# coecms/xmhw

Hardware: AMD Instinct MI355X
Metric: grid-cells/sec for threshold() on 40yr daily SST (higher is better)
Workload: dtype f32 in / f64 out; 1 GPU; 0.25deg global (configs[2]): 1036800 cells per step, 1982-2021 (T=14610), windowHalfWidth=5, pctile=90, smoothPercentileWidth=31, nan_frac=0.0, skipna=False; cells_rank0=1036800, T=14610, D=366, kernel=clim_sorted_f32 (sorted row-lists in LDS, 2 lanes per cell, layout 40), slabs=1, gather=none

## Files before the change

include/xmhw_amd.h:

```cpp
#ifndef XMHW_AMD_H
#define XMHW_AMD_H

#include <stddef.h>
#include <stdint.h>

#ifdef __cplusplus
extern "C" {
#endif

#define XMHW_OK 0
#define XMHW_ERR_INVALID 1
#define XMHW_ERR_HIP 2
#define XMHW_ERR_UNSUPPORTED 3
#define XMHW_ERR_NOMEM 4
#define XMHW_ERR_COMM 5

#define XMHW_KERNEL_AUTO 0
#define XMHW_KERNEL_RING 1
#define XMHW_KERNEL_GENERIC 2

int xmhw_version(void);
const char *xmhw_arch(void);
const char *xmhw_last_error(void);
int xmhw_device_count(int *count);
// ... 39 lines not shown
int xmhw_event_elapsed_ms(void *start, void *stop, float *ms);

typedef struct xmhw_plan xmhw_plan;

int xmhw_plan_create(const int32_t *doy_host, int64_t T, int32_t window_half_width,
                     xmhw_plan **plan);
int xmhw_plan_destroy(xmhw_plan *plan);
int xmhw_plan_info(const xmhw_plan *plan, int32_t *D, int32_t *ntracks,
                   int32_t *kernel, int32_t *nsteps, int32_t *step_min);
int xmhw_plan_doys(const xmhw_plan *plan, int32_t *doys_out );
int xmhw_plan_set_kernel(xmhw_plan *plan, int32_t kernel);
int xmhw_plan_set_narrowing(xmhw_plan *plan, int32_t enable);
int xmhw_plan_set_timing(xmhw_plan *plan, int32_t enable);
int xmhw_plan_kernel_ms(xmhw_plan *plan, int32_t calls_back, float *ms);
int xmhw_plan_narrowed(xmhw_plan *plan, int32_t *narrowed_out);
int xmhw_plan_set_chunks(xmhw_plan *plan, int32_t nchunks);
int xmhw_plan_chunks_in_use(const xmhw_plan *plan, int64_t C, int32_t *nchunks);
int xmhw_plan_table(const xmhw_plan *plan, int32_t years_per_lane, uint32_t *table_out,
                    int32_t *ntracks_padded);
int xmhw_plan_sorted_info(const xmhw_plan *plan, int64_t C, int32_t *keys_per_list, int32_t *lds_bytes_per_wave,
                          int32_t *pieces);
int xmhw_plan_sorted_table(const xmhw_plan *plan, int32_t pieces, int32_t *nchunks, int32_t *nrows, int32_t *ntp,
                           int32_t *chunks_out, uint32_t *table_out, uint32_t *flags_out);

int xmhw_debug_stats_available(void);
int xmhw_plan_debug_stats_n(xmhw_plan *plan, int enable, uint64_t *out, int32_t n);
int xmhw_plan_debug_stats(xmhw_plan *plan, int enable, uint64_t *out8);

enum {
    XMHW_LAYOUT_AUTO = -2,
    XMHW_LAYOUT_RING1 = -1,
    XMHW_LAYOUT_RING2_8LANE = 8,
    XMHW_LAYOUT_RING2_4LANE = 10,
    XMHW_LAYOUT_RING2_16LANE = 12,
    XMHW_LAYOUT_RING3_8LANE = 20,
    XMHW_LAYOUT_RING3_4LANE = 21,
    XMHW_LAYOUT_RING3_2LANE = 22,
    XMHW_LAYOUT_SORTED = 40
};
int xmhw_plan_set_layout(xmhw_plan *plan, int32_t layout);
int xmhw_plan_layout_in_use(const xmhw_plan *plan, int32_t *layout);
int xmhw_sorted_device_ok(int32_t *holds);
int xmhw_plan_set_ring2(xmhw_plan *plan, int32_t variant);
int xmhw_plan_ring2_in_use(const xmhw_plan *plan, int32_t *variant);
int xmhw_plan_f64_mode(const xmhw_plan *plan, int32_t *variant);
enum { XMHW_ROUTE_GENERIC = 0, XMHW_ROUTE_RING1 = 1, XMHW_ROUTE_RING2 = 2, XMHW_ROUTE_RING3 = 3, XMHW_ROUTE_RING4 = 4,
// ... 488 lines not shown
```

xmhw_amd/csrc/capi.cpp:

```cpp
#include "../../include/xmhw_amd.h"

#include <hip/hip_runtime.h>
#include <unistd.h>

#include <cerrno>
#include <cmath>

#include <algorithm>
#include <cstdio>
#include <cstdlib>
#include <atomic>
#include <cstring>
#include <map>
#include <memory>
#include <mutex>
#include <new>
#include <string>
#include <vector>

#include "kernels.h"
#include "plan.h"
#include "route.h"
#include "stage_blocks.h"

// ... 17 lines not shown
namespace {
#define HIP_TRY(expr)                                        \
    do {                                                     \
        hipError_t _e = (expr);                              \
        if (_e != hipSuccess) return hip_fail(_e, #expr);    \
    } while (0)

constexpr int kSubs = 8;

}

struct PlanDevice {
    int32_t* row_ptr = nullptr;
    int32_t* centres = nullptr;
    uint32_t* sflags = nullptr;
    xmhw::DevChunk* chunks = nullptr;
    int32_t nchunks = 0;
    unsigned long long* stats = nullptr;
    uint32_t* narrow_flag = nullptr;
    uint32_t* table_s = nullptr;
    uint32_t* sflags_s = nullptr;
    xmhw::DevSortedChunk* chunks_s = nullptr;
    int32_t nchunks_s = 0;
};

struct xmhw_plan {
    xmhw::Plan host;
    xmhw::RouteSettings settings = xmhw::route_defaults();
    std::mutex mu;
    bool uploaded = false;
    PlanDevice dev;
    std::map<std::pair<int32_t, int32_t>, uint32_t*> tables;
    int32_t chunks_cut = 0;
    int32_t yps_s = 0;
    int64_t sorted_pieces = -1;
    bool timing = false;
    hipEvent_t tev[32] = {};
    uint64_t tcalls = 0;

    ~xmhw_plan() {
        for (hipEvent_t e : tev) if (e) (void)hipEventDestroy(e);
        for (auto& kv : tables) if (kv.second) (void)hipFree(kv.second);
        for (void* p : std::initializer_list<void*>{dev.row_ptr, dev.centres, dev.sflags, dev.chunks, dev.stats,
                                                    dev.narrow_flag, dev.table_s, dev.sflags_s, dev.chunks_s})
            if (p) (void)hipFree(p);
    }
// ... 27 lines not shown
        r = xmhw::resolve_route(p->host, p->settings, elem_bytes, q, false);
    return r;
}
xmhw::Route plan_route(const xmhw_plan* p, int elem_bytes, double q = 1.0) {
    return xmhw::resolve_route(p->host, p->settings, elem_bytes, q, true);
}

template <typename E>
hipError_t put(E** dst, const std::vector<E>& v) {
    const bool fresh = *dst == nullptr;
    hipError_t e = fresh ? hipMalloc(reinterpret_cast<void**>(dst), sizeof(E) * v.size()) : hipSuccess;
    if (e != hipSuccess) { *dst = nullptr; return e; }
    e = hipMemcpy(*dst, v.data(), sizeof(E) * v.size(), hipMemcpyHostToDevice);
    if (e != hipSuccess && fresh) { (void)hipFree(*dst); *dst = nullptr; }
    return e;
}

struct Ready {
    PlanDevice dev;
    const uint32_t* table[3] = {};
    hipEvent_t t0 = nullptr, t1 = nullptr;
};

int ensure_sorted(xmhw_plan* p, const xmhw::Launch& l, int64_t pieces) {
    PlanDevice& d = p->dev;
    if (d.table_s && p->yps_s == l.tpl && p->sorted_pieces == pieces) return XMHW_OK;
    HIP_TRY(hipDeviceSynchronize());
    for (void** q : {reinterpret_cast<void**>(&d.table_s), reinterpret_cast<void**>(&d.sflags_s),
                     reinterpret_cast<void**>(&d.chunks_s)})
        if (*q) { HIP_TRY(hipFree(*q)); *q = nullptr; }
    const xmhw::Plan::SortedPlan sp = p->host.sorted_plan(l.lanes * l.tpl, 24, pieces);
    if (sp.chunks.empty()) return fail(XMHW_ERR_UNSUPPORTED, "the sorted-list kernel has no chunks for this plan");
    std::vector<xmhw::DevSortedChunk> cs(sp.chunks.size());
    for (size_t i = 0; i < cs.size(); ++i) cs[i] = {sp.chunks[i].warm_start, sp.chunks[i].begin, sp.chunks[i].end, sp.chunks[i].trow0};
    std::stable_sort(cs.begin(), cs.end(), [](const xmhw::DevSortedChunk& a, const xmhw::DevSortedChunk& b) {
        return a.end - a.warm_start > b.end - b.warm_start;
    });
    p->sorted_pieces = -1;
    HIP_TRY(put(&d.table_s, sp.table));
    HIP_TRY(put(&d.sflags_s, sp.flags));
    HIP_TRY(put(&d.chunks_s, cs));
    d.nchunks_s = static_cast<int32_t>(cs.size());
    p->yps_s = l.tpl;
    p->sorted_pieces = pieces;
    return XMHW_OK;
}

int ensure(xmhw_plan* p, const xmhw::Route& route, int64_t C, bool timed, Ready* out) {
    std::lock_guard<std::mutex> lock(p->mu);
    const xmhw::Plan& h = p->host;
    PlanDevice& d = p->dev;
    if (!p->uploaded) {
        HIP_TRY(put(&d.row_ptr, h.row_ptr));
        HIP_TRY(put(&d.centres, h.centres));
        HIP_TRY(put(&d.sflags, h.step_flags()));
        p->uploaded = true;
    }
// ... 54 lines not shown
    if (l.family == xmhw::Family::Ring2)
        return xmhw::launch_ring2_f32_narrowing(ts, C, ld, h.T, table, rd.sflags, h.step_min, rd.chunks, rd.nchunks, h.w,
                                                l.tpl, h.ntracks, l.layout, q, negate, thresh, seas, ldo, st, rd.narrow_flag);
    if (l.family == xmhw::Family::Ring3)
        return xmhw::launch_ring3_f32_narrowing(ts, C, ld, h.T, table, rd.sflags, h.step_min, rd.chunks, rd.nchunks, h.w,
                                                l.tpl, l.lanes, h.ntracks, q, negate, thresh, seas, ldo, st, rd.narrow_flag);
    return hipErrorInvalidValue;
}

template <typename T>
hipError_t launch_one(const xmhw::Plan& h, const xmhw::Launch& l, const PlanDevice& rd, const uint32_t* table, const T* ts,
                      int64_t C, int64_t ld, double q, int negate, double* thresh, double* seas, int64_t ldo,
                      hipStream_t st) {
    using xmhw::Family;
    const uint32_t* run_flag = l.gated ? rd.narrow_flag : nullptr;
    unsigned long long* stats = l.counters ? rd.stats : nullptr;
    if (l.family == Family::Generic)
        return xmhw::launch_generic<T>(ts, h.T, C, ld, rd.row_ptr, rd.centres, h.D, h.w, q, negate, thresh, seas, ldo, st,
                                       run_flag);
    if constexpr (sizeof(T) == 4) {
        switch (l.family) {
            case Family::Sorted:
                return xmhw::launch_sorted_f32(ts, C, ld, h.T, table, rd.sflags_s, rd.chunks_s, rd.nchunks_s, h.w, l.tpl,
                                               h.ntracks, q, negate, thresh, seas, ldo, st, stats);
            case Family::Ring1:
                return xmhw::launch_ring_f32(ts, C, ld, table, h.step_min, rd.chunks, rd.nchunks, h.w, l.tpl, l.lanes, q,
                                             negate, thresh, seas, ldo, st, stats);
            case Family::Ring2:
                return xmhw::launch_ring2_f32(ts, C, ld, h.T, table, rd.sflags, h.step_min, rd.chunks, rd.nchunks, h.w, l.tpl,
                                              h.ntracks, l.layout, q, negate, thresh, seas, ldo, st, stats);
            case Family::Ring3:
                return xmhw::launch_ring3_f32(ts, C, ld, h.T, table, rd.sflags, h.step_min, rd.chunks, rd.nchunks, h.w, l.tpl,
                                              l.lanes, h.ntracks, q, negate, thresh, seas, ldo, st, stats);
#ifdef XMHW_RING4
            case Family::Ring4:
                return xmhw::launch_ring4_f32(ts, C, ld, h.T, table, rd.sflags, h.step_min, rd.chunks, rd.nchunks, h.w, l.tpl,
                                              l.lanes, h.ntracks, q, negate, thresh, seas, ldo, st, stats);
#endif
            default: return hipErrorInvalidValue;
        }
    } else {
        if (l.narrows) return launch_narrowing(h, l, rd, table, ts, C, ld, q, negate, thresh, seas, ldo, st);
        if (l.family == Family::Ring2)
            return xmhw::launch_ring2_f64(ts, C, ld, h.T, table, rd.sflags, h.step_min, rd.chunks, rd.nchunks, h.w, l.tpl,
                                          h.ntracks, l.layout, q, negate, thresh, seas, ldo, st, run_flag);
        if (l.family == Family::Ring3)
            return xmhw::launch_ring3_f64(ts, C, ld, h.T, table, rd.sflags, h.step_min, rd.chunks, rd.nchunks, h.w, l.tpl,
// ... 1367 lines not shown
}

int xmhw_plan_sorted_table(const xmhw_plan* plan, int32_t pieces, int32_t* nchunks, int32_t* nrows, int32_t* ntp,
                           int32_t* chunks_out, uint32_t* table_out, uint32_t* flags_out) {
    if (!plan) return fail(XMHW_ERR_INVALID, "plan is NULL");
    const int32_t yps = xmhw::sorted_pick_yps(plan->host.w, plan->host.ntracks);
    if (yps == 0) return fail(XMHW_ERR_UNSUPPORTED, "the sorted-list kernel is not instantiated for this window / record length");
    const xmhw::Plan::SortedPlan sp = plan->host.sorted_plan(2 * yps, 24, std::max(pieces, 1));
    if (nchunks) *nchunks = static_cast<int32_t>(sp.chunks.size());
    if (nrows) *nrows = static_cast<int32_t>(sp.flags.size());
    if (ntp) *ntp = 2 * yps;
    if (chunks_out)
        for (size_t i = 0; i < sp.chunks.size(); ++i) {
            chunks_out[4 * i + 0] = sp.chunks[i].warm_start;
            chunks_out[4 * i + 1] = sp.chunks[i].begin;
            chunks_out[4 * i + 2] = sp.chunks[i].end;
            chunks_out[4 * i + 3] = sp.chunks[i].trow0;
        }
    if (table_out) std::memcpy(table_out, sp.table.data(), sizeof(uint32_t) * sp.table.size());
    if (flags_out) std::memcpy(flags_out, sp.flags.data(), sizeof(uint32_t) * sp.flags.size());
    return XMHW_OK;
}

int xmhw_clim_raw_f32(xmhw_plan* plan, const float* ts, int64_t C, int64_t ld, double q, int negate,
                      double* thresh, double* seas, int64_t ldo, void* stream) {
    return clim_raw<float>(plan, ts, C, ld, q, negate, thresh, seas, ldo, stream);
}
int xmhw_clim_raw_f64(xmhw_plan* plan, const double* ts, int64_t C, int64_t ld, double q, int negate,
                      double* thresh, double* seas, int64_t ldo, void* stream) {
    return clim_raw<double>(plan, ts, C, ld, q, negate, thresh, seas, ldo, stream);
}

int xmhw_clim_raw_i16(xmhw_plan* plan, const int16_t* codes, int64_t C, int64_t ld, int big_endian, int has_scale,
                      double scale_factor, double add_offset, int has_fill, int32_t fill_code, int decoded_itemsize, double q,
                      int negate, double* thresh, double* seas, int64_t ldo, void* stream) {
    if (!plan) return fail(XMHW_ERR_INVALID, "plan is NULL");
    if (C < 0 || ld < C || ldo < C) return fail(XMHW_ERR_INVALID, "bad C/ld/ldo");
    if (!(q >= 0.0 && q <= 1.0)) return fail(XMHW_ERR_INVALID, "quantile must be in [0, 1]");
    if (decoded_itemsize != 4 && decoded_itemsize != 8) return fail(XMHW_ERR_INVALID, "decoded_itemsize must be 4 or 8");
    if (has_scale && !(scale_factor == scale_factor && add_offset == add_offset && scale_factor != 0.0))
        return fail(XMHW_ERR_INVALID, "scale_factor must be a non-zero number, add_offset a number");
    if (C == 0) return XMHW_OK;
    if (!codes || !thresh || !seas) return fail(XMHW_ERR_INVALID, "NULL device buffer");
    const xmhw::Route route = call_route(plan, 4, q);
    if (!route.n || route.launch[0].family != xmhw::Family::Sorted)
        return fail(XMHW_ERR_UNSUPPORTED, "packed input runs on the sorted-list kernel only (w = 5, 9..48 tracks, quantile >= 0.85 or <= 0.15): "
// ... 932 lines not shown
```

xmhw_amd/csrc/kernels.h:

```cpp
#pragma once
#include <hip/hip_runtime.h>
#include <stdint.h>

namespace xmhw {

struct DevChunk { int32_t warm_start, begin, end; };
struct PackedI16 {
    int32_t mode = 0;
    int32_t fill = 0x7FFFFFFF;
    int32_t swap = 0;
    int32_t key_neg = 0;
    int32_t val_neg = 0;
    float sf = 1.0f, of = 0.0f;
    double s = 1.0, o = 0.0;
};
struct DevSortedChunk { int32_t warm_start, begin, end, trow0; };

template <typename T>
hipError_t launch_generic(const T* ts, int64_t Tn, int64_t C, int64_t ld, const int32_t* row_ptr,
                          const int32_t* centres, int32_t D, int32_t w, double q, int negate,
                          double* thresh, double* seas, int64_t ldo, hipStream_t stream,
                          const uint32_t* run_flag = nullptr);

bool ring_supported(int32_t w, int32_t yps, int32_t subs, int elem_bytes);
int32_t ring_pick(int32_t w, int32_t ntracks, int elem_bytes, int32_t* subs_out);
hipError_t launch_ring_f32(const float* ts, int64_t C, int64_t ld, const uint32_t* table,
                           int32_t step_min, const DevChunk* chunks, int32_t nchunks,
                           int32_t w, int32_t yps, int32_t subs, double q, int negate, double* thresh,
                           double* seas, int64_t ldo, hipStream_t stream,
                           unsigned long long* stats = nullptr);

int32_t ring2_pick_yps(int32_t w, int32_t ntracks, int32_t variant);
bool ring2_narrowing_supported(int32_t w, int32_t yps, int32_t variant);
hipError_t launch_narrow_probe(const double* ts, int64_t Tn, int64_t C, int64_t ld, uint32_t* narrow_flag, hipStream_t stream);
hipError_t launch_ring2_f32_narrowing(const double* ts, int64_t C, int64_t ld, int64_t Tn, const uint32_t* table,
                                      const uint32_t* sflags, int32_t step_min, const DevChunk* chunks,
                                      int32_t nchunks, int32_t w, int32_t yps, int32_t ntracks, int32_t variant,
                                      double q, int negate, double* thresh, double* seas, int64_t ldo,
                                      hipStream_t stream, uint32_t* narrow_flag);
// ... 5 lines not shown
                            double* thresh, double* seas, int64_t ldo, hipStream_t stream, const uint32_t* run_flag);
bool ring_stats_built();
hipError_t launch_ring2_f32(const float* ts, int64_t C, int64_t ld, int64_t Tn, const uint32_t* table,
                            const uint32_t* sflags, int32_t step_min, const DevChunk* chunks, int32_t nchunks,
                            int32_t w, int32_t yps, int32_t ntracks, int32_t variant, double q, int negate,
                            double* thresh, double* seas, int64_t ldo, hipStream_t stream,
                            unsigned long long* stats = nullptr);

int32_t ring3_pick_yps(int32_t w, int32_t ntracks, int32_t subs);
bool ring3_supported(int32_t w, int32_t yps, int32_t subs);
hipError_t launch_ring3_f32(const float* ts, int64_t C, int64_t ld, int64_t Tn, const uint32_t* table,
                            const uint32_t* sflags, int32_t step_min, const DevChunk* chunks, int32_t nchunks,
                            int32_t w, int32_t yps, int32_t subs, int32_t ntracks, double q, int negate,
                            double* thresh, double* seas, int64_t ldo, hipStream_t stream,
                            unsigned long long* stats = nullptr);

int32_t sorted_pick_yps(int32_t w, int32_t ntracks);
int32_t sorted_pick_k(int32_t w, int32_t ntracks);
int32_t sorted_lds_bytes(int32_t w, int32_t ntracks);
hipError_t sorted_lds_probe(uint32_t* d_bad, hipStream_t stream);
hipError_t launch_sorted_f32(const float* ts, int64_t C, int64_t ld, int64_t Tn, const uint32_t* table,
                             const uint32_t* sflags, const DevSortedChunk* chunks, int32_t nchunks,
                             int32_t w, int32_t yps, int32_t ntracks, double q, int negate, double* thresh, double* seas,
                             int64_t ldo, hipStream_t stream, unsigned long long* stats = nullptr);
hipError_t launch_sorted_i16(const int16_t* codes, const PackedI16& pk, int64_t C, int64_t ld, int64_t Tn,
                             const uint32_t* table, const uint32_t* sflags, const DevSortedChunk* chunks, int32_t nchunks,
                             int32_t w, int32_t yps, int32_t ntracks, double q, int negate, double* thresh, double* seas,
                             int64_t ldo, hipStream_t stream);

int32_t ring4_pick_yps(int32_t w, int32_t ntracks, int32_t subs);
bool ring4_supported(int32_t w, int32_t yps, int32_t subs);
bool ring4_stats_built();
hipError_t launch_ring4_f32(const float* ts, int64_t C, int64_t ld, int64_t Tn, const uint32_t* table,
                            const uint32_t* sflags, int32_t step_min, const DevChunk* chunks, int32_t nchunks,
                            int32_t w, int32_t yps, int32_t subs, int32_t ntracks, double q, int negate,
                            double* thresh, double* seas, int64_t ldo, hipStream_t stream,
                            unsigned long long* stats = nullptr);

bool ring3_x64_supported(int32_t w, int32_t yps, int32_t subs);
hipError_t launch_ring3_f64(const double* ts, int64_t C, int64_t ld, int64_t Tn, const uint32_t* table,
                            const uint32_t* sflags, int32_t step_min, const DevChunk* chunks, int32_t nchunks,
                            int32_t w, int32_t yps, int32_t subs, int32_t ntracks, double q, int negate, double* thresh,
                            double* seas, int64_t ldo, hipStream_t stream, const uint32_t* run_flag);
bool ring3_narrowing_supported(int32_t w, int32_t yps, int32_t subs);
hipError_t launch_ring3_f32_narrowing(const double* ts, int64_t C, int64_t ld, int64_t Tn, const uint32_t* table,
                                      const uint32_t* sflags, int32_t step_min, const DevChunk* chunks,
                                      int32_t nchunks, int32_t w, int32_t yps, int32_t subs, int32_t ntracks, double q,
// ... 359 lines not shown
```

xmhw_amd/csrc/kernels_sorted.hip:

```cpp
#include <type_traits>

#include "device_common.h"
#include "kernels.h"
#include "packed_src.h"
#include "plan.h"
#include "sorted_count.h"
#include "sortnet_gen.h"

namespace xmhw {
namespace {

typedef __attribute__((address_space(3))) uint32_t lds_u32;
__device__ __forceinline__ uint32_t lds_ld(uint32_t a) { return *reinterpret_cast<lds_u32*>(static_cast<uintptr_t>(a)); }
__device__ __forceinline__ void lds_st(uint32_t a, uint32_t v) { *reinterpret_cast<lds_u32*>(static_cast<uintptr_t>(a)) = v; }

constexpr int kSwap1 = 0xB1;
__device__ __forceinline__ uint32_t swp(uint32_t v) {
    return static_cast<uint32_t>(__builtin_amdgcn_update_dpp(0, static_cast<int>(v), kSwap1, 0xF, 0xF, true));
}
__device__ __forceinline__ double swp(double v) {
    const uint64_t b = static_cast<uint64_t>(__double_as_longlong(v));
    const uint32_t lo = swp(static_cast<uint32_t>(b)), hi = swp(static_cast<uint32_t>(b >> 32));
    return __longlong_as_double(static_cast<long long>((static_cast<uint64_t>(hi) << 32) | lo));
}
// ... 149 lines not shown
                ev = count_eq(v);
            }
        }
    }
    if (!found) {
        v = 0;
        for (int bit = 31; bit >= 0; --bit) {
            const uint32_t cand = v | (1u << bit);
            uint32_t cnt = 0;
#pragma unroll
            for (int i = 0; i < KPL; ++i)
                cnt += static_cast<uint32_t>(__builtin_popcountll(__builtin_amdgcn_ballot_w64(key[i] - 1u < cand - 1u)));
            if (cnt <= lo) v = cand;
        }
        cl = count_lt(v);
        ev = count_eq(v);
    }
    uint32_t vhi = v;
    if (lo + 1 < n && lo + 1 >= cl + ev) vhi = next_above(v);
    out_lo = v;
    out_hi = vhi;
}

}

template <int YPS, int K, int KL, bool STATS, bool PACKED>
__device__ __forceinline__ void sorted_body(
    const void* __restrict__ ts, int64_t C, int64_t ld, int64_t Tn, const uint32_t* __restrict__ table,
    const uint32_t* __restrict__ sflags, const DevSortedChunk* __restrict__ chunks, double q, int negate,
    int32_t ntracks, double* __restrict__ thresh, double* __restrict__ seas, int64_t ldo,
    unsigned long long* __restrict__ stats, const PackedI16& pk) {
    constexpr int R = 11;
    constexpr uint32_t ES = PACKED ? 2u : 4u;
    constexpr int NL = 6;
    constexpr int HE = (YPS + 1) / 2 * 2;
    constexpr int HH = HE / 2;
    constexpr int KH = K / 2;
#ifndef XMHW_SERIAL_MAX
#define XMHW_SERIAL_MAX 3
#endif
    constexpr uint32_t kSerialMax = XMHW_SERIAL_MAX;
    constexpr int NTP = 2 * YPS;
    constexpr uint32_t LSTRIDE = 32 * 4;
    constexpr uint32_t RSTRIDE = R * LSTRIDE;
    constexpr int LDS_BYTES = (R * KL * static_cast<int>(LSTRIDE) + kLdsGranule - 1) / kLdsGranule * kLdsGranule;
    static_assert(K <= HE && K % 2 == 0, "a list stores an even number of keys, at most what a lane holds");
    constexpr int EXT = K - KL;
    static_assert(EXT == 0 || ((EXT == 2 || EXT == 4) && KL >= KH), "two or four register ranks, all from lane 1's half");
    constexpr int EXN = EXT > 0 ? EXT : 1;
    static_assert(LDS_BYTES == 8960 || LDS_BYTES == 11520 || LDS_BYTES == 14080 || LDS_BYTES == 17920 || LDS_BYTES == 20480 ||
                  LDS_BYTES == 23040 || LDS_BYTES == 25600, "sorted_lds_probe() checks these allocation sizes");
    __shared__ __attribute__((aligned(16))) uint32_t lds[LDS_BYTES / 4];

    const int lane = threadIdx.x & 63;
    const int sub = lane & 1;
    const int cw = lane >> 1;
    const int64_t cell = static_cast<int64_t>(blockIdx.x) * 32 + cw;
    const bool cell_ok = cell < C;
    const DevSortedChunk ch = chunks[blockIdx.y];
    const int32_t step_min = ch.warm_start - ch.trow0;
    const char* col = static_cast<const char*>(ts) + (cell_ok ? cell : C - 1) * static_cast<int64_t>(ES);
    const bool mirror = q < 0.5;
    const int kneg = (negate != 0) != mirror ? 1 : 0;
    const uint32_t tmax = static_cast<uint32_t>(Tn - 1);
    const bool padded_last = (YPS - 1) * 2 + sub >= ntracks;
    const uint32_t padmask = padded_last ? 0xFFFFFFFFu : 0u;
    const uint32_t* tab = table + sub;

    const uint32_t lds0 = static_cast<uint32_t>(reinterpret_cast<uintptr_t>((lds_u32*)lds));
    if (lds0 != 0u) __builtin_trap();
    const uint32_t lcell = static_cast<uint32_t>(cw) * 4u;
    for (int i = lane; i < LDS_BYTES / 4; i += 64) lds[i] = 0u;
    __builtin_amdgcn_s_waitcnt(0);
    __builtin_amdgcn_wave_barrier();

    uint32_t P[NL];
    V32 TV = 0;
#define XMHW_RSLO(j) TV[2 * (j)]
#define XMHW_RSHI(j) TV[2 * (j) + 1]
#define XMHW_EX(e, j) TV[12 + 6 * (e) + (j)]
#define XMHW_NVL(j) TV[24 + (j)]
    uint32_t lbase[NL];
#pragma unroll
    for (int j = 0; j < NL; ++j) {
        const int g = sub * NL + j;
        lbase[j] = g < R ? lcell + static_cast<uint32_t>(g) * LSTRIDE : 0x40000000u + lcell;
        P[j] = 0;
    }
    static_assert(KL >= 5, "a list holds a window");
    static_assert(NL == 6 && EXT <= 2, "the register vector holds five values of six lists");
// ... 725 lines not shown
        }
        tick(4);
        sf_cur = sf_nxt;
        sf_nxt = __builtin_amdgcn_readfirstlane(sf_nn);
    }
    if (ep_s >= 0) finish_rows();
    if (STATS && stats != nullptr) {
        if (lane == 0) {
            atomicAdd(&stats[0], static_cast<unsigned long long>(st_rows));
            atomicAdd(&stats[1], static_cast<unsigned long long>(st_iter));
#pragma unroll
            for (int i = 1; i < 4; ++i) atomicAdd(&stats[4 + i], static_cast<unsigned long long>(st_more[i]));
            atomicAdd(&stats[4], static_cast<unsigned long long>(st_ext));
#pragma unroll
            for (int i = 0; i < 8; ++i) atomicAdd(&stats[8 + i], tacc[i]);
        }
        if (sub == 0) {
            atomicAdd(&stats[2], static_cast<unsigned long long>(st_flag));
            atomicAdd(&stats[3], static_cast<unsigned long long>(st_steps));
        }
    }
}

#ifndef XMHW_WAVES3_MAX_YPS
#define XMHW_WAVES3_MAX_YPS 8
#endif
#define XMHW_WAVES_PER_SIMD(Y) ((Y) <= XMHW_WAVES3_MAX_YPS ? 3 : 2)
template <int YPS, int K, int KL, bool STATS>
__global__ __launch_bounds__(64, XMHW_WAVES_PER_SIMD(YPS)) void clim_sorted_f32(
    const float* __restrict__ ts, int64_t C, int64_t ld, int64_t Tn, const uint32_t* __restrict__ table,
    const uint32_t* __restrict__ sflags, const DevSortedChunk* __restrict__ chunks, double q, int negate,
    int32_t ntracks, double* __restrict__ thresh, double* __restrict__ seas, int64_t ldo,
    unsigned long long* __restrict__ stats) {
    sorted_body<YPS, K, KL, STATS, false>(ts, C, ld, Tn, table, sflags, chunks, q, negate, ntracks, thresh, seas, ldo, stats,
                                      PackedI16{});
}
template <int YPS, int K, int KL>
__global__ __launch_bounds__(64, XMHW_WAVES_PER_SIMD(YPS)) void clim_sorted_i16(
    const int16_t* __restrict__ codes, PackedI16 pk, int64_t C, int64_t ld, int64_t Tn, const uint32_t* __restrict__ table,
    const uint32_t* __restrict__ sflags, const DevSortedChunk* __restrict__ chunks, double q, int negate,
    int32_t ntracks, double* __restrict__ thresh, double* __restrict__ seas, int64_t ldo) {
    sorted_body<YPS, K, KL, false, true>(codes, C, ld, Tn, table, sflags, chunks, q, negate, ntracks, thresh, seas, ldo, nullptr, pk);
}

namespace {
typedef void (*SortedKernel)(const float*, int64_t, int64_t, int64_t, const uint32_t*, const uint32_t*,
                             const DevSortedChunk*, double, int, int32_t, double*, double*, int64_t, unsigned long long*);
typedef void (*SortedKernelI16)(const int16_t*, PackedI16, int64_t, int64_t, int64_t, const uint32_t*, const uint32_t*,
                                const DevSortedChunk*, double, int, int32_t, double*, double*, int64_t);
struct SortedEntry { int yps, k, kl; SortedKernel fn, fn_stats; SortedKernelI16 fn_i16; };
#ifdef XMHW_RING_STATS
#define XMHW_SS(Y, K, KL) clim_sorted_f32<Y, K, KL, true>
#else
#define XMHW_SS(Y, K, KL) nullptr
#endif
#define XMHW_S2(Y, K, KL) {Y, K, KL, clim_sorted_f32<Y, K, KL, false>, XMHW_SS(Y, K, KL), clim_sorted_i16<Y, K, KL>}
#define XMHW_S(Y, K) XMHW_S2(Y, K, K)
#ifndef XMHW_K40
#define XMHW_K40 16
#endif
#ifndef XMHW_KL48
#define XMHW_KL48 16
#endif
#ifndef XMHW_KL40
#define XMHW_KL40 14
#endif
const SortedEntry kSorted[] = {
#ifdef XMHW_SORTED_ONLY
    XMHW_S2(20, XMHW_K40, XMHW_KL40),
#else
    XMHW_S(5, 6),   XMHW_S(6, 6),   XMHW_S(7, 8),   XMHW_S(8, 8),   XMHW_S(9, 10),  XMHW_S(10, 10), XMHW_S(11, 10),
    XMHW_S(12, 10), XMHW_S(13, 12), XMHW_S(14, 12), XMHW_S(15, 12), XMHW_S(16, 12), XMHW_S(17, 14), XMHW_S(18, 14),
    XMHW_S2(19, XMHW_K40, XMHW_KL40), XMHW_S2(20, XMHW_K40, XMHW_KL40), XMHW_S2(21, 18, XMHW_KL48), XMHW_S2(22, 18, XMHW_KL48), XMHW_S2(23, 18, XMHW_KL48), XMHW_S2(24, 18, XMHW_KL48),
#endif
};
#undef XMHW_S
#undef XMHW_S2
#undef XMHW_SS
const SortedEntry* find_sorted(int32_t yps) {
// ... 36 lines not shown
}

int32_t sorted_pick_yps(int32_t w, int32_t ntracks) {
    if (w != 5) return 0;
    const int32_t yps = (ntracks + 1) / 2;
    return find_sorted(yps) ? yps : 0;
}

int32_t sorted_pick_k(int32_t w, int32_t ntracks) {
    if (w != 5) return 0;
    const SortedEntry* e = find_sorted((ntracks + 1) / 2);
    return e ? e->k : 0;
}

int32_t sorted_lds_bytes(int32_t w, int32_t ntracks) {
    if (w != 5) return 0;
    const SortedEntry* e = find_sorted((ntracks + 1) / 2);
    return e ? (11 * e->kl * 128 + kLdsGranule - 1) / kLdsGranule * kLdsGranule : 0;
}

hipError_t launch_sorted_f32(const float* ts, int64_t C, int64_t ld, int64_t Tn, const uint32_t* table,
                             const uint32_t* sflags, const DevSortedChunk* chunks, int32_t nchunks,
                             int32_t w, int32_t yps, int32_t ntracks, double q, int negate, double* thresh, double* seas,
                             int64_t ldo, hipStream_t stream, unsigned long long* stats) {
    const SortedEntry* e = w == 5 ? find_sorted(yps) : nullptr;
    if (!e || ld >= (int64_t(1) << 30)) return hipErrorInvalidValue;
    if (C <= 0 || nchunks <= 0) return hipSuccess;
    dim3 grid(static_cast<unsigned>((C + 31) / 32), static_cast<unsigned>(nchunks));
    const bool twin = stats != nullptr && e->fn_stats != nullptr;
    hipLaunchKernelGGL(twin ? e->fn_stats : e->fn, grid, dim3(64), 0, stream, ts, C, ld, Tn, table, sflags, chunks, q,
                       negate, ntracks, thresh, seas, ldo, twin ? stats : nullptr);
    return hipGetLastError();
}

hipError_t launch_sorted_i16(const int16_t* codes, const PackedI16& pk, int64_t C, int64_t ld, int64_t Tn,
                             const uint32_t* table, const uint32_t* sflags, const DevSortedChunk* chunks, int32_t nchunks,
                             int32_t w, int32_t yps, int32_t ntracks, double q, int negate, double* thresh, double* seas,
                             int64_t ldo, hipStream_t stream) {
    const SortedEntry* e = w == 5 ? find_sorted(yps) : nullptr;
    if (!e || !e->fn_i16 || ld >= (int64_t(1) << 30) || pk.mode < 1 || pk.mode > 3) return hipErrorInvalidValue;
    if (C <= 0 || nchunks <= 0) return hipSuccess;
    dim3 grid(static_cast<unsigned>((C + 31) / 32), static_cast<unsigned>(nchunks));
    hipLaunchKernelGGL(e->fn_i16, grid, dim3(64), 0, stream, codes, pk, C, ld, Tn, table, sflags, chunks, q, negate, ntracks,
                       thresh, seas, ldo);
    return hipGetLastError();
}

}
```

xmhw_amd/csrc/plan.cpp:

```cpp
#include "plan.h"

#include <algorithm>

namespace xmhw {

bool Plan::build(const int32_t* doy, int64_t T_, int32_t w_) {
    if (T_ <= 0) { error = "time axis is empty"; return false; }
    if (w_ < 0) { error = "windowHalfWidth must be >= 0"; return false; }
    if (T_ > (int64_t(1) << 30) - 4) { error = "time axis too long"; return false; }
    T = T_;
    w = w_;
    R = 2 * w + 1;
    doys.assign(doy, doy + T);
    std::sort(doys.begin(), doys.end());
    doys.erase(std::unique(doys.begin(), doys.end()), doys.end());
    D = static_cast<int32_t>(doys.size());
    row_of_t.resize(T);
    for (int64_t t = 0; t < T; ++t)
        row_of_t[t] = static_cast<int32_t>(std::lower_bound(doys.begin(), doys.end(), doy[t]) - doys.begin());
    track_begin.clear();
    track_end.clear();
    track_begin.push_back(0);
    for (int64_t t = 1; t < T; ++t) {
        if (doy[t] <= doy[t - 1]) {
// ... 148 lines not shown
                for (int32_t i = 1; i <= R - 1; ++i) {
                    uint32_t ent = make_entry(kCodeInvalid, true);
                    while (src > step_min) {
                        --src;
                        const uint32_t o = orig(src, k);
                        if ((o >> 1) != kCodeHold) { ent = o | 1u; break; }
                    }
                    out.table[base + static_cast<size_t>(b - i - ch.warm_start) * ntp + k] = ent;
                }
            }
            for (int32_t v = 0; v < nrows; ++v) {
                bool simple = true, consec = v > 0;
                for (int32_t k = 0; k < ntracks; ++k) {
                    const uint32_t en = out.table[base + static_cast<size_t>(v) * ntp + k];
                    simple = simple && (en >> 1) >= 2u;
                    if (v > 0) {
                        const uint32_t pr = out.table[base + static_cast<size_t>(v - 1) * ntp + k];
                        consec = consec && (en >> 1) >= 2u && (pr >> 1) >= 2u && (en >> 1) == (pr >> 1) + 1u;
                    }
                }
                out.flags.push_back((simple ? 1u : 0u) | (consec ? 2u : 0u));
            }
            out.chunks.push_back(ch);
        }
    }
    return out;
}

}
```

xmhw_amd/csrc/plan.h:

```cpp
#pragma once
#include <cstdint>
#include <string>
#include <vector>

namespace xmhw {

constexpr uint32_t kCodeHold = 0;
constexpr uint32_t kCodeInvalid = 1;
constexpr uint32_t make_entry(uint32_t code, bool counted) { return (code << 1) | (counted ? 1u : 0u); }

struct Chunk {
    int32_t warm_start;
    int32_t begin;
    int32_t end;
};

struct Plan {
    int64_t T = 0;
    int32_t w = 0;
    int32_t R = 1;
    int32_t D = 0;
    std::vector<int32_t> doys;
    std::vector<int32_t> row_of_t;
    int32_t ntracks = 0;
    std::vector<int64_t> track_begin, track_end;
    std::vector<int32_t> row_ptr;
    std::vector<int32_t> centres;
    int32_t max_centres = 0;
    int32_t step_min = 0;
    int32_t nsteps = 0;
    int32_t nchunks_req = 0;

    std::string error;

    bool build(const int32_t* doy, int64_t T, int32_t w);
    std::vector<uint32_t> ring_table(int32_t subs, int32_t yps) const;
    std::vector<uint32_t> step_flags() const;
    std::vector<Chunk> make_chunks(int32_t nchunks) const;
    int32_t warm_start_for(int32_t begin) const;
    struct SortedChunk { int32_t warm_start, begin, end, trow0; };
    struct SortedPlan {
        std::vector<SortedChunk> chunks;
        std::vector<uint32_t> table, flags;
    };
    SortedPlan sorted_plan(int32_t ntp, int32_t min_rows_per_piece, int64_t pieces_wanted) const;
};

}
```

xmhw_amd/csrc/pybind.cpp:

```cpp
#include "pybind_common.h"

PYBIND11_MODULE(_xmhw_hip, m) {
    m.doc() = "C-ABI bindings of the gfx950 xmhw threshold() path";
    auto& hip_error = py::register_exception<HipError>(m, "HipError");
    py::register_exception<Unsupported>(m, "Unsupported", hip_error.ptr());
    py::register_exception<InvalidError>(m, "InvalidArgument");
    py::register_exception<CommError>(m, "CommError");

    m.attr("KERNEL_AUTO") = XMHW_KERNEL_AUTO;
    m.attr("KERNEL_RING") = XMHW_KERNEL_RING;
    m.attr("KERNEL_GENERIC") = XMHW_KERNEL_GENERIC;

    m.def("version", &xmhw_version);
    m.def("arch", []() { return std::string(xmhw_arch()); });
    m.def("device_count", []() { int n = 0; check(xmhw_device_count(&n)); return n; });
    m.def("set_device", [](int d) { check(xmhw_set_device(d)); });
    m.def("get_device", []() { int d = 0; check(xmhw_get_device(&d)); return d; });
    m.def("device_info", [](int d) {
        char name[256] = {0};
        int cus = 0;
        uint64_t bytes = 0;
        check(xmhw_device_info(d, name, sizeof(name), &cus, &bytes));
        py::dict r;
        r["name"] = std::string(name);
// ... 64 lines not shown
        check(xmhw_plan_table(p, yps, nullptr, &ntp));
        py::array_t<uint32_t> out({static_cast<py::ssize_t>(ns), static_cast<py::ssize_t>(ntp)});
        check(xmhw_plan_table(p, yps, out.mutable_data(), &ntp));
        return out;
    });

    m.def("plan_set_timing", [](Ptr p, int on) { check(xmhw_plan_set_timing(p, on)); });
    m.def("plan_kernel_ms", [](Ptr p, int back) { float ms = 0; check(xmhw_plan_kernel_ms(p, back, &ms)); return ms; });
    m.def("plan_sorted_info", [](Ptr p, int64_t C) {
        int32_t k = 0, lds = 0, pieces = 0;
        check(xmhw_plan_sorted_info(p, C, &k, &lds, &pieces));
        return py::make_tuple(k, lds, pieces);
    });
    m.def("plan_sorted_table", [](Ptr p, int pieces) {
        int32_t nc = 0, nr = 0, ntp = 0;
        check(xmhw_plan_sorted_table(p, pieces, &nc, &nr, &ntp, nullptr, nullptr, nullptr));
        py::array_t<int32_t> chunks({static_cast<py::ssize_t>(nc), static_cast<py::ssize_t>(4)});
        py::array_t<uint32_t> table({static_cast<py::ssize_t>(nr), static_cast<py::ssize_t>(ntp)});
        py::array_t<uint32_t> flags(static_cast<py::ssize_t>(nr));
        check(xmhw_plan_sorted_table(p, pieces, &nc, &nr, &ntp, chunks.mutable_data(), table.mutable_data(),
                                     flags.mutable_data()));
        return py::make_tuple(chunks, table, flags);
    });

    m.def("plan_debug_stats", [](Ptr p, int enable, bool read) {
        py::array_t<uint64_t> out(16);
        std::fill(out.mutable_data(), out.mutable_data() + 16, uint64_t(0));
        check(xmhw_plan_debug_stats_n(p, enable, read ? out.mutable_data() : nullptr, 16));
        return out;
    });
    m.def("plan_chunks_in_use", [](Ptr p, int64_t C) { int32_t v = 0; check(xmhw_plan_chunks_in_use(p, C, &v)); return v; });
    m.def("debug_stats_available", []() { return xmhw_debug_stats_available() != 0; });
    m.def("plan_set_layout", [](Ptr p, int layout) { check(xmhw_plan_set_layout(p, layout)); });
    m.def("plan_layout_in_use", [](Ptr p) { int32_t v = -1; check(xmhw_plan_layout_in_use(p, &v)); return v; });
    m.def("sorted_device_ok", []() { int32_t v = 0; check(xmhw_sorted_device_ok(&v)); return v != 0; });
    m.def("plan_f64_mode", [](Ptr p) { int32_t v = -1; check(xmhw_plan_f64_mode(p, &v)); return v; });
    m.def("plan_route", [](Ptr p, int elem_bytes, double q, int64_t C) {
        py::array_t<int32_t> out(XMHW_ROUTE_WORDS);
        check(xmhw_plan_route(p, elem_bytes, q, C, out.mutable_data(), XMHW_ROUTE_WORDS));
        return out;
    });

    m.def("clim_raw", [](Ptr plan, Ptr ts, int itemsize, int64_t C, int64_t ld, double q, int negate, Ptr th, Ptr se,
                         int64_t ldo, Ptr stream) {
        check(by_itemsize(itemsize, xmhw_clim_raw_f32, xmhw_clim_raw_f64, plan, ts, C, ld, q, negate, th, se, ldo, stream));
    }, py::arg("plan"), py::arg("ts"), py::arg("itemsize"), py::arg("C"), py::arg("ld"), py::arg("q"),
// ... 458 lines not shown
```

xmhw_amd/device.py:

```python
import os as _os
import sys
import threading as _threading
import time as _time
from concurrent.futures import ThreadPoolExecutor
from contextlib import contextmanager

import numpy as np

from ._lib import hip
from .exception import XmhwException

KERNELS = {"auto": 0, "ring": 1, "generic": 2}


class PackedArray(np.ndarray):

    def __new__(cls, array, decode):
        obj = np.asarray(array).view(cls)
        obj.decode = dict(decode)
        return obj

    def __array_finalize__(self, obj):
        if obj is not None:
            self.decode = getattr(obj, "decode", None)
# ... 200 lines not shown
        self.T = doy.shape[0]
        self.w = int(window_half_width)

    def layout_in_use(self):
        return int(self._h.plan_layout_in_use(self.handle))

    ring2_in_use = layout_in_use

    def chunks_in_use(self, C):
        return int(self._h.plan_chunks_in_use(self.handle, int(C)))

    def f64_mode(self):
        return int(self._h.plan_f64_mode(self.handle))

    def route(self, dtype, q, C=1):
        r = [int(v) for v in self._h.plan_route(self.handle, np.dtype(dtype).itemsize, float(q), int(C))]
        keys = ("family", "layout", "lanes", "tracks_per_lane", "narrows", "gated", "counters")
        launches = [dict(zip(keys, r[2 + 7 * i:9 + 7 * i])) for i in range(r[1])]
        for la in launches:
            la["family"] = ROUTE_FAMILIES[la["family"]]
            for k in keys[4:]:
                la[k] = bool(la[k])
        return {"supported": r[0] == 0, "launches": launches, "chunks": r[23], "sorted_pieces": r[24]}

    def narrowed(self):
        return bool(self._h.plan_narrowed(self.handle))

    def table(self, years_per_lane):
        return self._h.plan_table(self.handle, years_per_lane)

    def destroy(self):
        if getattr(self, "handle", 0):
            self._h.plan_destroy(self.handle)
            self.handle = 0

    def __del__(self):
        try:
            self.destroy()
        except Exception:
            pass


def _first_family(route):
    return route["launches"][0]["family"] if route["launches"] else None


# ... 530 lines not shown
```

Baseline: 43.05 million cells/s.

## Compute single-row sorted chunks directly with register sorting networks

Chunks of the sorted-list plan that cover one output row with a small pooled track set are flagged at plan time. They are then handled by a direct path that gathers the 11 window rows, sorts them in registers and picks the percentile, instead of maintaining LDS sorted lists with warm-up rows. For small years-per-lane a separate one-row kernel is launched before the main kernel, and the main kernel returns early for those chunks. The aim is to remove warm-up and incremental-update work for chunks that produce only one row. The cost is an extra launch and higher register pressure in the direct path.

```diff
diff --git a/include/xmhw_amd.h b/include/xmhw_amd.h
--- a/include/xmhw_amd.h
+++ b/include/xmhw_amd.h
@@ -85,6 +85,7 @@
                           int32_t *pieces);
 int xmhw_plan_sorted_table(const xmhw_plan *plan, int32_t pieces, int32_t *nchunks, int32_t *nrows, int32_t *ntp,
                            int32_t *chunks_out, uint32_t *table_out, uint32_t *flags_out);
+int xmhw_plan_sorted_direct(const xmhw_plan *plan, int64_t C, int32_t *count);
 
 int xmhw_debug_stats_available(void);
 int xmhw_plan_debug_stats_n(xmhw_plan *plan, int enable, uint64_t *out, int32_t n);
diff --git a/xmhw_amd/csrc/capi.cpp b/xmhw_amd/csrc/capi.cpp
--- a/xmhw_amd/csrc/capi.cpp
+++ b/xmhw_amd/csrc/capi.cpp
@@ -63,6 +63,7 @@
     uint32_t* sflags_s = nullptr;
     xmhw::DevSortedChunk* chunks_s = nullptr;
     int32_t nchunks_s = 0;
+    int32_t ndirect_s = 0;
 };
 
 struct xmhw_plan {
@@ -136,6 +137,14 @@
     hipEvent_t t0 = nullptr, t1 = nullptr;
 };
 
+bool sorted_onerow_enabled() {
+    static const bool on = [] {
+        const char* v = std::getenv("XMHW_SORTED_ONEROW");
+        return !(v && v[0] == '0' && v[1] == '\0');
+    }();
+    return on;
+}
+
 int ensure_sorted(xmhw_plan* p, const xmhw::Launch& l, int64_t pieces) {
     PlanDevice& d = p->dev;
     if (d.table_s && p->yps_s == l.tpl && p->sorted_pieces == pieces) return XMHW_OK;
@@ -146,7 +155,14 @@
     const xmhw::Plan::SortedPlan sp = p->host.sorted_plan(l.lanes * l.tpl, 24, pieces);
     if (sp.chunks.empty()) return fail(XMHW_ERR_UNSUPPORTED, "the sorted-list kernel has no chunks for this plan");
     std::vector<xmhw::DevSortedChunk> cs(sp.chunks.size());
-    for (size_t i = 0; i < cs.size(); ++i) cs[i] = {sp.chunks[i].warm_start, sp.chunks[i].begin, sp.chunks[i].end, sp.chunks[i].trow0};
+    const bool onerow = sorted_onerow_enabled();
+    d.ndirect_s = 0;
+    for (size_t i = 0; i < cs.size(); ++i) {
+        const uint64_t set = onerow && sp.direct(i, xmhw::sorted_direct_tracks(l.tpl)) ? sp.pooled[i] : 0;
+        d.ndirect_s += set != 0 ? 1 : 0;
+        cs[i] = {sp.chunks[i].warm_start, sp.chunks[i].begin, sp.chunks[i].end, sp.chunks[i].trow0,
+                 static_cast<uint32_t>(set), static_cast<uint32_t>(set >> 32)};
+    }
     std::stable_sort(cs.begin(), cs.end(), [](const xmhw::DevSortedChunk& a, const xmhw::DevSortedChunk& b) {
         return a.end - a.warm_start > b.end - b.warm_start;
     });
@@ -247,7 +263,7 @@
         switch (l.family) {
             case Family::Sorted:
                 return xmhw::launch_sorted_f32(ts, C, ld, h.T, table, rd.sflags_s, rd.chunks_s, rd.nchunks_s, h.w, l.tpl,
-                                               h.ntracks, q, negate, thresh, seas, ldo, st, stats);
+                                               h.ntracks, q, negate, thresh, seas, ldo, st, stats, rd.ndirect_s);
             case Family::Ring1:
                 return xmhw::launch_ring_f32(ts, C, ld, table, h.step_min, rd.chunks, rd.nchunks, h.w, l.tpl, l.lanes, q,
                                              negate, thresh, seas, ldo, st, stats);
@@ -1661,6 +1677,18 @@
     return XMHW_OK;
 }
 
+int xmhw_plan_sorted_direct(const xmhw_plan* plan, int64_t C, int32_t* count) {
+    if (!plan || !count) return fail(XMHW_ERR_INVALID, "NULL argument");
+    if (C < 0) return fail(XMHW_ERR_INVALID, "bad C");
+    const int32_t yps = xmhw::sorted_pick_yps(plan->host.w, plan->host.ntracks);
+    if (yps == 0) return fail(XMHW_ERR_UNSUPPORTED, "the sorted-list kernel is not instantiated for this window / record length");
+    const xmhw::Plan::SortedPlan sp = plan->host.sorted_plan(2 * yps, 24, xmhw::sorted_pieces(plan->host, plan_route(plan, 4), C));
+    int32_t n = 0;
+    for (size_t i = 0; i < sp.chunks.size(); ++i) n += sorted_onerow_enabled() && sp.direct(i, xmhw::sorted_direct_tracks(yps)) ? 1 : 0;
+    *count = n;
+    return XMHW_OK;
+}
+
 int xmhw_clim_raw_f32(xmhw_plan* plan, const float* ts, int64_t C, int64_t ld, double q, int negate,
                       double* thresh, double* seas, int64_t ldo, void* stream) {
     return clim_raw<float>(plan, ts, C, ld, q, negate, thresh, seas, ldo, stream);
diff --git a/xmhw_amd/csrc/kernels.h b/xmhw_amd/csrc/kernels.h
--- a/xmhw_amd/csrc/kernels.h
+++ b/xmhw_amd/csrc/kernels.h
@@ -14,7 +14,7 @@
     float sf = 1.0f, of = 0.0f;
     double s = 1.0, o = 0.0;
 };
-struct DevSortedChunk { int32_t warm_start, begin, end, trow0; };
+struct DevSortedChunk { int32_t warm_start, begin, end, trow0; uint32_t direct_lo, direct_hi; };
 
 template <typename T>
 hipError_t launch_generic(const T* ts, int64_t Tn, int64_t C, int64_t ld, const int32_t* row_ptr,
@@ -66,7 +66,8 @@
 hipError_t launch_sorted_f32(const float* ts, int64_t C, int64_t ld, int64_t Tn, const uint32_t* table,
                              const uint32_t* sflags, const DevSortedChunk* chunks, int32_t nchunks,
                              int32_t w, int32_t yps, int32_t ntracks, double q, int negate, double* thresh, double* seas,
-                             int64_t ldo, hipStream_t stream, unsigned long long* stats = nullptr);
+                             int64_t ldo, hipStream_t stream, unsigned long long* stats = nullptr,
+                             int32_t ndirect = 0);
 hipError_t launch_sorted_i16(const int16_t* codes, const PackedI16& pk, int64_t C, int64_t ld, int64_t Tn,
                              const uint32_t* table, const uint32_t* sflags, const DevSortedChunk* chunks, int32_t nchunks,
                              int32_t w, int32_t yps, int32_t ntracks, double q, int negate, double* thresh, double* seas,
diff --git a/xmhw_amd/csrc/kernels_sorted.hip b/xmhw_amd/csrc/kernels_sorted.hip
--- a/xmhw_amd/csrc/kernels_sorted.hip
+++ b/xmhw_amd/csrc/kernels_sorted.hip
@@ -195,6 +195,171 @@
     out_hi = vhi;
 }
 
+#ifndef XMHW_WAVES3_MAX_YPS
+#define XMHW_WAVES3_MAX_YPS 8
+#endif
+#if XMHW_WAVES3_MAX_YPS == 8
+static_assert(sorted_direct_tracks(8) == 6 && sorted_direct_tracks(9) == 12, "the three-wave builds settle 6 tracks directly (plan.h)");
+#endif
+constexpr bool direct_in_launch(int yps) { return yps > XMHW_WAVES3_MAX_YPS; }
+
+template <int N>
+__device__ __forceinline__ void direct_top(uint32_t (&a)[N], const uint32_t (&b)[N]) {
+    if constexpr (N == 12) {
+        uint32_t v[2 * N];
+#pragma unroll
+        for (int i = 0; i < N; ++i) { v[i] = a[i]; v[N + i] = b[i]; }
+        sortnet::MergeTop<N, N, N>::run(v);
+#pragma unroll
+        for (int i = 0; i < N; ++i) a[i] = v[i];
+    } else {
+        constexpr int H = N / 2;
+        uint32_t hi[H], lo[H];
+#pragma unroll
+        for (int i = 0; i < H; ++i) {
+            const uint32_t p = umax(a[i], b[N - 1 - i]), r = umax(a[i + H], b[H - 1 - i]);
+            hi[i] = umax(p, r);
+            lo[i] = umin(p, r);
+        }
+        sortnet::BitonicDesc<H>::run(hi);
+        sortnet::BitonicDesc<H>::run(lo);
+#pragma unroll
+        for (int i = 0; i < H; ++i) { a[i] = hi[i]; a[H + i] = lo[i]; }
+    }
+}
+
+template <int NTP, int NT>
+__device__ __forceinline__ void direct_row(const char* __restrict__ col, bool cell_ok, int64_t cell, int sub, uint32_t ld4,
+                                           uint32_t tmax, const uint32_t* __restrict__ table, const DevSortedChunk& ch,
+                                           double q, int negate, bool mirror, int kneg, double* __restrict__ thresh,
+                                           double* __restrict__ seas, int64_t ldo) {
+    constexpr int R = 11, NS = 6, NK = 2 * NT;
+    static_assert(NT == 6 || NT == 12, "the sorters below are those of 6 / 12 and 12 / 24 keys");
+    uint64_t set = (static_cast<uint64_t>(ch.direct_hi) << 32) | ch.direct_lo;
+    uint32_t kt[NT], here[NT], even[NT], odd[NT];
+    const uint32_t k_first = static_cast<uint32_t>(__builtin_ctzll(set));
+#pragma unroll
+    for (int i = 0; i < NT; ++i) {
+        const bool have = set != 0ull;
+        kt[i] = have ? static_cast<uint32_t>(__builtin_ctzll(set)) : k_first;
+        here[i] = have ? 0xFFFFFFFFu : 0u;
+        odd[i] = here[i] & (0u - (kt[i] & 1u));
+        even[i] = here[i] & ~odd[i];
+        set &= set - 1ull;
+    }
+    const int m0 = ((ch.warm_start % R) + R) % R;
+    uint32_t rowi[NS];
+    uint32_t stepm[NS];
+#pragma unroll
+    for (int j = 0; j < NS; ++j) {
+        const int g = sub * NS + j;
+        stepm[j] = g < R ? 0xFFFFFFFFu : 0u;
+        int off = g - m0;
+        off = off < 0 ? off + R : off;
+        off = g < R ? off : 0;
+        rowi[j] = static_cast<uint32_t>(ch.trow0 + off) * static_cast<uint32_t>(NTP);
+    }
+    uint32_t ent[NT][NS];
+#pragma unroll
+    for (int i = 0; i < NT; ++i)
+#pragma unroll
+        for (int j = 0; j < NS; ++j) ent[i][j] = table[rowi[j] + kt[i]];
+    float x[NT][NS];
+#pragma unroll
+    for (int i = 0; i < NT; ++i)
+#pragma unroll
+        for (int j = 0; j < NS; ++j) {
+            ent[i][j] = XMHW_BITOP3(ent[i][j], stepm[j], here[i], 0x80);
+            const uint32_t t = umin((ent[i][j] >> 1) - 2u, tmax);
+            x[i][j] = *reinterpret_cast<const float*>(col + static_cast<uint64_t>(t) * ld4);
+        }
+    __builtin_amdgcn_s_waitcnt(0);
+    __builtin_amdgcn_sched_barrier(0);
+    const uint32_t kflip = kneg ? 0x80000000u : 0u;
+    uint32_t key[NS][NT];
+    double d_even[NS], d_odd[NS];
+    uint32_t nv = 0;
+#pragma unroll
+    for (int j = 0; j < NS; ++j) d_even[j] = d_odd[j] = 0.0;
+#pragma unroll
+    for (int i = 0; i < NT; ++i) {
+#pragma unroll
+        for (int j = 0; j < NS; ++j) {
+            const float v = x[i][j];
+            const uint32_t bits = __float_as_uint(v);
+            const uint32_t okm = (v == v && ent[i][j] >= 4u) ? 0xFFFFFFFFu : 0u;
+            key[j][i] = key_fast<false>(bits ^ kflip) & okm;
+            nv -= okm;
+            d_even[j] += static_cast<double>(__uint_as_float(XMHW_BITOP3(bits, okm, even[i], 0x80)));
+            d_odd[j] += static_cast<double>(__uint_as_float(XMHW_BITOP3(bits, okm, odd[i], 0x80)));
+        }
+    }
+    double tsum = 0.0;
+#pragma unroll
+    for (int j = 0; j < NS; ++j) {
+        const double de = negate ? -d_even[j] : d_even[j], dd = negate ? -d_odd[j] : d_odd[j];
+        tsum += de + dd;
+    }
+    const double total = tsum + swp(tsum);
+    const uint32_t n = nv + swp(nv);
+    uint32_t top[NK];
+    {
+        uint32_t r01[NK], r23[NK], r45[NK];
+#pragma unroll
+        for (int j = 0; j < NS; ++j) sort_desc<NT>(key[j]);
+#pragma unroll
+        for (int i = 0; i < NT; ++i) {
+            r01[i] = key[0][i]; r01[NT + i] = key[1][i];
+            r23[i] = key[2][i]; r23[NT + i] = key[3][i];
+            r45[i] = key[4][i]; r45[NT + i] = key[5][i];
+        }
+        sortnet::MergeTop<NT, NT, NK>::run(r01);
+        sortnet::MergeTop<NT, NT, NK>::run(r23);
+        sortnet::MergeTop<NT, NT, NK>::run(r45);
+        direct_top(r01, r23);
+        direct_top(r01, r45);
+        uint32_t oth[NK];
+#pragma unroll
+        for (int i = 0; i < NK; ++i) oth[i] = swp(r01[i]);
+        direct_top(r01, oth);
+#pragma unroll
+        for (int i = 0; i < NK; ++i) top[i] = r01[i];
+    }
+    const uint32_t nn = n ? n : 1u;
+    const double vi = static_cast<double>(nn - 1) * q;
+    const double fl = floor(vi);
+    const double g = vi - fl;
+    const uint32_t lo = static_cast<uint32_t>(fl);
+    const bool need2 = lo + 1 < nn;
+    const uint32_t Cs = n ? (mirror ? lo + 1u : n - 1u - lo) : 0u;
+    uint32_t a_lo = 0u, a_hi = 0u;
+#pragma unroll
+    for (int i = 0; i < NK; ++i) {
+        a_lo = Cs == static_cast<uint32_t>(i) ? top[i] : a_lo;
+        a_hi = Cs == static_cast<uint32_t>(i + 1) ? top[i] : a_hi;
+    }
+    if (!need2) {
+        if (mirror) a_lo = a_hi;
+        else a_hi = a_lo;
+    }
+    double th = make_nan(), se = make_nan();
+    if (n > 0) {
+        double v_lo = static_cast<double>(key_f32(mirror ? a_hi : a_lo));
+        double v_hi = static_cast<double>(key_f32(mirror ? a_lo : a_hi));
+        if (mirror) {
+            v_lo = -v_lo;
+            v_hi = -v_hi;
+        }
+        se = total / static_cast<double>(n);
+        th = numpy_lerp(v_lo, v_hi, g);
+    }
+    if (sub == 0 && cell_ok) {
+        const int64_t row = static_cast<int64_t>(ch.begin);
+        thresh[row * ldo + cell] = th;
+        seas[row * ldo + cell] = se;
+    }
+}
+
 }
 
 template <int YPS, int K, int KL, bool STATS, bool PACKED>
@@ -239,6 +404,15 @@
     const bool padded_last = (YPS - 1) * 2 + sub >= ntracks;
     const uint32_t padmask = padded_last ? 0xFFFFFFFFu : 0u;
     const uint32_t* tab = table + sub;
+
+    if constexpr (!PACKED && !STATS) {
+        if ((ch.direct_lo | ch.direct_hi) != 0u) {
+            if constexpr (direct_in_launch(YPS))
+                direct_row<NTP, sorted_direct_tracks(YPS)>(col, cell_ok, cell, sub, static_cast<uint32_t>(ld) * ES, tmax, table, ch, q,
+                                                           negate, mirror, kneg, thresh, seas, ldo);
+            return;
+        }
+    }
 
     const uint32_t lds0 = static_cast<uint32_t>(reinterpret_cast<uintptr_t>((lds_u32*)lds));
     if (lds0 != 0u) __builtin_trap();
@@ -1010,9 +1184,6 @@
     }
 }
 
-#ifndef XMHW_WAVES3_MAX_YPS
-#define XMHW_WAVES3_MAX_YPS 8
-#endif
 #define XMHW_WAVES_PER_SIMD(Y) ((Y) <= XMHW_WAVES3_MAX_YPS ? 3 : 2)
 template <int YPS, int K, int KL, bool STATS>
 __global__ __launch_bounds__(64, XMHW_WAVES_PER_SIMD(YPS)) void clim_sorted_f32(
@@ -1023,6 +1194,23 @@
     sorted_body<YPS, K, KL, STATS, false>(ts, C, ld, Tn, table, sflags, chunks, q, negate, ntracks, thresh, seas, ldo, stats,
                                       PackedI16{});
 }
+template <int YPS>
+__global__ __launch_bounds__(64) void sorted_onerow_f32(
+    const float* __restrict__ ts, int64_t C, int64_t ld, int64_t Tn, const uint32_t* __restrict__ table,
+    const DevSortedChunk* __restrict__ chunks, double q, int negate, double* __restrict__ thresh, double* __restrict__ seas,
+    int64_t ldo) {
+    const DevSortedChunk ch = chunks[blockIdx.y];
+    if ((ch.direct_lo | ch.direct_hi) == 0u) return;
+    const int lane = threadIdx.x & 63;
+    const int sub = lane & 1;
+    const int64_t cell = static_cast<int64_t>(blockIdx.x) * 32 + (lane >> 1);
+    const bool cell_ok = cell < C;
+    const char* col = reinterpret_cast<const char*>(ts) + (cell_ok ? cell : C - 1) * 4;
+    const bool mirror = q < 0.5;
+    const int kneg = (negate != 0) != mirror ? 1 : 0;
+    direct_row<2 * YPS, sorted_direct_tracks(YPS)>(col, cell_ok, cell, sub, static_cast<uint32_t>(ld) * 4u, static_cast<uint32_t>(Tn - 1),
+                                                   table, ch, q, negate, mirror, kneg, thresh, seas, ldo);
+}
 template <int YPS, int K, int KL>
 __global__ __launch_bounds__(64, XMHW_WAVES_PER_SIMD(YPS)) void clim_sorted_i16(
     const int16_t* __restrict__ codes, PackedI16 pk, int64_t C, int64_t ld, int64_t Tn, const uint32_t* __restrict__ table,
@@ -1036,13 +1224,20 @@
                              const DevSortedChunk*, double, int, int32_t, double*, double*, int64_t, unsigned long long*);
 typedef void (*SortedKernelI16)(const int16_t*, PackedI16, int64_t, int64_t, int64_t, const uint32_t*, const uint32_t*,
                                 const DevSortedChunk*, double, int, int32_t, double*, double*, int64_t);
-struct SortedEntry { int yps, k, kl; SortedKernel fn, fn_stats; SortedKernelI16 fn_i16; };
+typedef void (*SortedOnerow)(const float*, int64_t, int64_t, int64_t, const uint32_t*, const DevSortedChunk*, double, int,
+                             double*, double*, int64_t);
+template <int YPS>
+constexpr SortedOnerow onerow_of() {
+    if constexpr (direct_in_launch(YPS)) return nullptr;
+    else return sorted_onerow_f32<YPS>;
+}
+struct SortedEntry { int yps, k, kl; SortedKernel fn, fn_stats; SortedKernelI16 fn_i16; SortedOnerow fn_onerow; };
 #ifdef XMHW_RING_STATS
 #define XMHW_SS(Y, K, KL) clim_sorted_f32<Y, K, KL, true>
 #else
 #define XMHW_SS(Y, K, KL) nullptr
 #endif
-#define XMHW_S2(Y, K, KL) {Y, K, KL, clim_sorted_f32<Y, K, KL, false>, XMHW_SS(Y, K, KL), clim_sorted_i16<Y, K, KL>}
+#define XMHW_S2(Y, K, KL) {Y, K, KL, clim_sorted_f32<Y, K, KL, false>, XMHW_SS(Y, K, KL), clim_sorted_i16<Y, K, KL>, onerow_of<Y>()}
 #define XMHW_S(Y, K) XMHW_S2(Y, K, K)
 #ifndef XMHW_K40
 #define XMHW_K40 16
@@ -1125,12 +1320,14 @@
 hipError_t launch_sorted_f32(const float* ts, int64_t C, int64_t ld, int64_t Tn, const uint32_t* table,
                              const uint32_t* sflags, const DevSortedChunk* chunks, int32_t nchunks,
                              int32_t w, int32_t yps, int32_t ntracks, double q, int negate, double* thresh, double* seas,
-                             int64_t ldo, hipStream_t stream, unsigned long long* stats) {
+                             int64_t ldo, hipStream_t stream, unsigned long long* stats, int32_t ndirect) {
     const SortedEntry* e = w == 5 ? find_sorted(yps) : nullptr;
     if (!e || ld >= (int64_t(1) << 30)) return hipErrorInvalidValue;
     if (C <= 0 || nchunks <= 0) return hipSuccess;
     dim3 grid(static_cast<unsigned>((C + 31) / 32), static_cast<unsigned>(nchunks));
     const bool twin = stats != nullptr && e->fn_stats != nullptr;
+    if (ndirect > 0 && e->fn_onerow != nullptr && !twin)
+        hipLaunchKernelGGL(e->fn_onerow, grid, dim3(64), 0, stream, ts, C, ld, Tn, table, chunks, q, negate, thresh, seas, ldo);
     hipLaunchKernelGGL(twin ? e->fn_stats : e->fn, grid, dim3(64), 0, stream, ts, C, ld, Tn, table, sflags, chunks, q,
                        negate, ntracks, thresh, seas, ldo, twin ? stats : nullptr);
     return hipGetLastError();
diff --git a/xmhw_amd/csrc/plan.cpp b/xmhw_amd/csrc/plan.cpp
--- a/xmhw_amd/csrc/plan.cpp
+++ b/xmhw_amd/csrc/plan.cpp
@@ -194,9 +194,23 @@
                 out.flags.push_back((simple ? 1u : 0u) | (consec ? 2u : 0u));
             }
             out.chunks.push_back(ch);
+            uint64_t set = 0;
+            for (int32_t k = 0; k < ntracks && k < 64; ++k) set |= inS[k] ? uint64_t(1) << k : 0;
+            out.pooled.push_back(set);
         }
     }
     return out;
 }
 
-}
+bool Plan::SortedPlan::direct(size_t i, int32_t max_tracks) const {
+    const SortedChunk& ch = chunks[i];
+    if (ch.end - ch.begin != 1) return false;
+    int32_t npool = 0;
+    for (uint64_t s = pooled[i]; s; s &= s - 1) ++npool;
+    if (npool < 1 || npool > max_tracks) return false;
+    for (int32_t v = 0; v < ch.end - ch.warm_start; ++v)
+        if (flags[static_cast<size_t>(ch.trow0 + v)] & 1u) return false;
+    return true;
+}
+
+}
diff --git a/xmhw_amd/csrc/plan.h b/xmhw_amd/csrc/plan.h
--- a/xmhw_amd/csrc/plan.h
+++ b/xmhw_amd/csrc/plan.h
@@ -8,6 +8,8 @@
 constexpr uint32_t kCodeHold = 0;
 constexpr uint32_t kCodeInvalid = 1;
 constexpr uint32_t make_entry(uint32_t code, bool counted) { return (code << 1) | (counted ? 1u : 0u); }
+
+constexpr int32_t sorted_direct_tracks(int32_t tracks_per_lane) { return tracks_per_lane <= 8 ? 6 : 12; }
 
 struct Chunk {
     int32_t warm_start;
@@ -42,6 +44,8 @@
     struct SortedPlan {
         std::vector<SortedChunk> chunks;
         std::vector<uint32_t> table, flags;
+        std::vector<uint64_t> pooled;
+        bool direct(size_t chunk, int32_t max_tracks) const;
     };
     SortedPlan sorted_plan(int32_t ntp, int32_t min_rows_per_piece, int64_t pieces_wanted) const;
 };
diff --git a/xmhw_amd/csrc/pybind.cpp b/xmhw_amd/csrc/pybind.cpp
--- a/xmhw_amd/csrc/pybind.cpp
+++ b/xmhw_amd/csrc/pybind.cpp
@@ -110,6 +110,7 @@
                                      flags.mutable_data()));
         return py::make_tuple(chunks, table, flags);
     });
+    m.def("_plan_sorted_direct", [](Ptr p, int64_t C) { int32_t v = 0; check(xmhw_plan_sorted_direct(p, C, &v)); return v; });
 
     m.def("plan_debug_stats", [](Ptr p, int enable, bool read) {
         py::array_t<uint64_t> out(16);
diff --git a/xmhw_amd/device.py b/xmhw_amd/device.py
--- a/xmhw_amd/device.py
+++ b/xmhw_amd/device.py
@@ -246,6 +246,10 @@
             for k in keys[4:]:
                 la[k] = bool(la[k])
         return {"supported": r[0] == 0, "launches": launches, "chunks": r[23], "sorted_pieces": r[24]}
+
+    def sorted_direct(self, C=1):
+        with as_xmhw_errors():
+            return int(self._h._plan_sorted_direct(self.handle, int(C)))
 
     def narrowed(self):
         return bool(self._h.plan_narrowed(self.handle))
```

Measured after the change: 44.00 million cells/s (median of 6 runs). 2.2% higher.
